# JuliaDiff/FiniteDiff.jl

Measured on AMD Instinct MI355X. Metric: Jacobian columns/s (coloured sparse finite-difference Jacobian; headline config N=10^7 tridiagonal forward), higher is better.
Workload: dtype f64; 1 GPU; N=10000000 tridiagonal CSC (nnz=3N-2), colorvec=mod1(i,3), forward, f!=second difference, x~U(0,1) seed 4; fdtype=forward, colors=3, parallelism=columns x1, output=nzval in HBM, eps_reduction=replicated, x_layout=replicated, gather_in_step=False

## Files before the change

finitediff.jl_amd/csrc/fdjac_builtin_f.hip:

```cpp
#include <atomic>
#include <cstdlib>
#include <mutex>
#include <new>
#include <unordered_map>
#include <vector>

#include "fdjac_internal.h"
#include "fdjac_eps_dev.h"

namespace fdjac {

constexpr real_t kTwo = 2, kFour = 4;
struct cd {
    real_t re, im;
};
__device__ __forceinline__ cd operator+(cd a, cd b) { return {a.re + b.re, a.im + b.im}; }
__device__ __forceinline__ cd operator-(cd a, cd b) { return {a.re - b.re, a.im - b.im}; }
__device__ __forceinline__ cd operator*(cd a, cd b) { return {a.re * b.re - a.im * b.im, a.re * b.im + a.im * b.re}; }
__device__ __forceinline__ cd operator*(real_t s, cd a) { return {s * a.re, s * a.im}; }
__device__ __forceinline__ cd operator+(cd a, real_t s) { return {a.re + s, a.im}; }
__device__ __forceinline__ cd operator-(cd a, real_t s) { return {a.re - s, a.im}; }

template <typename T> __device__ __forceinline__ T zero_of();
template <> __device__ __forceinline__ real_t zero_of<real_t>() { return 0.0; }
// ... 81 lines not shown
            xv[k] = in ? x[in ? j : 0] : 0.0;
            const int c = in ? (int)color[in ? j : 0] : -1;
            cv[k] = (c == (int)(CT)(-1) || c < 0) ? -1 : c - c_lo;
        }
        const bool two = i + 1 < n;
        real_t b0 = 0.0, b1 = 0.0;
        if (base_out || (diff && MODE == 0)) {
            b0 = tridiag_row<real_t, NL>(xv[0], xv[1], xv[2]);
            if (two) b1 = tridiag_row<real_t, NL>(xv[1], xv[2], xv[3]);
        }
        if (base_out) {
            if (two) *reinterpret_cast<r2_t *>(base_out + i) = r2_t{b0, b1};
            else base_out[i] = b0;
        }
        for (int b = 0; b < B; ++b) {
            const real_t e = eps[c_lo + b];
            real_t d[4];
#pragma unroll
            for (int k = 0; k < 4; ++k) d[k] = (cv[k] == b) ? e : 0.0;
            if (MODE == 2) {
                cd p[4];
#pragma unroll
                for (int k = 0; k < 4; ++k) p[k] = cd{xv[k], d[k]};
                const cd v0 = tridiag_row<cd, NL>(p[0], p[1], p[2]);
                if (imag_only) {
                    real_t *dst = fx + (int64_t)b * fs + i;
                    if (two) {
                        const cd v1 = tridiag_row<cd, NL>(p[1], p[2], p[3]);
                        *reinterpret_cast<r2_t *>(dst) = r2_t{v0.im, v1.im};
                    } else {
                        dst[0] = v0.im;
                    }
                } else {
                    real_t *dst = fx + ((int64_t)b * fs + i) * 2;
                    *reinterpret_cast<r2_t *>(dst) = r2_t{v0.re, v0.im};
                    if (two) {
                        const cd v1 = tridiag_row<cd, NL>(p[1], p[2], p[3]);
                        *reinterpret_cast<r2_t *>(dst + 2) = r2_t{v1.re, v1.im};
                    }
                }
            } else if (diff) {
                real_t p[4], q[4];
#pragma unroll
                for (int k = 0; k < 4; ++k) { p[k] = xv[k] + d[k]; q[k] = xv[k] - d[k]; }
                const real_t s0 = MODE == 1 ? tridiag_row<real_t, NL>(q[0], q[1], q[2]) : b0;
                const real_t v0 = sub_exact(tridiag_row<real_t, NL>(p[0], p[1], p[2]), s0);
                real_t v1 = 0.0;
                if (two) {
                    const real_t s1 = MODE == 1 ? tridiag_row<real_t, NL>(q[1], q[2], q[3]) : b1;
                    v1 = sub_exact(tridiag_row<real_t, NL>(p[1], p[2], p[3]), s1);
                }
                real_t *dst = fx + (int64_t)b * fs + i;
                if (two) *reinterpret_cast<r2_t *>(dst) = r2_t{v0, v1};
                else dst[0] = v0;
            } else {
#pragma unroll
                for (int sgn = 0; sgn < (MODE == 1 ? 2 : 1); ++sgn) {
                    real_t p[4];
#pragma unroll
                    for (int k = 0; k < 4; ++k) p[k] = sgn == 0 ? xv[k] + d[k] : xv[k] - d[k];
                    const real_t v0 = tridiag_row<real_t, NL>(p[0], p[1], p[2]);
                    real_t *dst = fx + (int64_t)(sgn * B + b) * fs + i;
                    if (two) {
                        const real_t v1 = tridiag_row<real_t, NL>(p[1], p[2], p[3]);
                        *reinterpret_cast<r2_t *>(dst) = r2_t{v0, v1};
                    } else {
                        dst[0] = v0;
                    }
                }
            }
        }
    }
}

__device__ __forceinline__ r2_t ld_pair_guarded(const real_t *__restrict__ x, int64_t a, int64_t n)
{
    if (a >= 0 && a + 1 < n) return *reinterpret_cast<const r2_t *>(x + a);
    r2_t v = {0, 0};
    if (a >= 0 && a < n) v.x = x[a];
    return v;
}

template <int MODE, bool NL>
__device__ __forceinline__ void tridiag_pair_quotients(const r2_t &L, const r2_t &Cc, const r2_t &R, real_t ea, real_t eb, real_t (&q)[6])
{
    const real_t xv[6] = {L.x, L.y, Cc.x, Cc.y, R.x, R.y};
#pragma unroll
    for (int o = 0; o < 2; ++o) {
        const real_t e = o == 0 ? ea : eb;
        const real_t ed = MODE == 1 ? 2 * e : e;
        real_t p[5], m[5];
#pragma unroll
        for (int k = 0; k < 5; ++k) { const real_t dlt = k == 2 ? e : (real_t)0; p[k] = xv[o + k] + dlt; m[k] = xv[o + k] - dlt; }
#pragma unroll
        for (int k = 0; k < 3; ++k) {
            const real_t plus = tridiag_row<real_t, NL>(p[k], p[k + 1], p[k + 2]);
            const real_t sub = MODE == 1 ? tridiag_row<real_t, NL>(m[k], m[k + 1], m[k + 2])
                                         : tridiag_row<real_t, NL>(xv[o + k], xv[o + k + 1], xv[o + k + 2]);
            q[3 * o + k] = sub_exact(plus, sub) / ed;
        }
    }
}

template <int MODE, bool NL>
__global__ void __launch_bounds__(kBlock)
k_f_tridiag_store_wave(const real_t *__restrict__ x, const real_t *__restrict__ eps, int64_t n, fd_band_store bst, int64_t jstart)
{
    __shared__ __attribute__((aligned(16))) real_t s_win[kBlock / 64][FD_BAND_WAVE_LDS(3)];
    const int lane = threadIdx.x & 63, wave = threadIdx.x >> 6;
    const int64_t nwaves = (bst.col_end - jstart + 127) / 128;
    const int64_t gw = (int64_t)blockIdx.x * (kBlock / 64) + wave;
    if (gw >= nwaves) return;
    const int64_t jw = jstart + gw * 128;
    const int64_t j = jw + 2 * lane;
    const r2_t Cc = ld_pair_guarded(x, j, n), L = ld_pair_guarded(x, j - 2, n), R = ld_pair_guarded(x, j + 2, n);
    const int c0w = (int)((jw + bst.shift) % bst.C);
    const int c0 = (int)((uint32_t)(c0w + 2 * lane) % (uint32_t)bst.C);
    const int c1 = c0 + 1 == bst.C ? 0 : c0 + 1;
    const real_t ea = eps[c0], eb = eps[c1];
    real_t q[6];
    tridiag_pair_quotients<MODE, NL>(L, Cc, R, ea, eb, q);
    fd_band_emit_wave<real_t, 3, true>(&bst, s_win[wave], jw, q);
}

template <int MODE, bool NL, int NC, bool PIPE>
__global__ void __launch_bounds__(kBlock)
k_f_tridiag_fused(const real_t *__restrict__ x, int64_t n, fd_band_store bst, int64_t jstart, FusedEps fz)
{
    constexpr int kWinBytes = (kBlock / 64) * FD_BAND_WAVE_LDS(3) * (int)sizeof(real_t);
    constexpr int kLdsBytes = kWinBytes + 64 > (kFzMaxBlocks + 2 * kEpsGroups) * 8 ? kWinBytes + 64 : (kFzMaxBlocks + 2 * kEpsGroups) * 8;
    __shared__ __attribute__((aligned(16))) char s_lds[kLdsBytes];
    real_t (*s_win)[FD_BAND_WAVE_LDS(3)] = reinterpret_cast<real_t (*)[FD_BAND_WAVE_LDS(3)]>(s_lds);
    double *s_red = reinterpret_cast<double *>(s_lds);
    const int b = (int)blockIdx.x, nfin = fz.eg.C;
    if (b < nfin) { fused_finisher(fz, b, s_red, x, n); return; }
    if (b < nfin + fz.nblocks) { fused_eps_block<NC, PIPE>(x, n, fz, b - nfin, reinterpret_cast<double (*)[NC]>(s_red)); return; }
    const int lane = threadIdx.x & 63, wave = threadIdx.x >> 6;
    const int cb = b - nfin - fz.nblocks;
    const int64_t nwaves = (bst.col_end - jstart + 127) / 128;
    const int64_t gstride = (int64_t)((int)gridDim.x - nfin - fz.nblocks) * (kBlock / 64);
    int64_t gw = (int64_t)cb * (kBlock / 64) + wave;
    int64_t jw = jstart + gw * 128;
    r2_t Cc = {0, 0}, L = {0, 0}, R = {0, 0};
    auto load_x = [&](int64_t jt, r2_t &c_, r2_t &l_, r2_t &r_) {
        const int64_t j = jt + 2 * lane;
        c_ = ld_pair_guarded(x, j, n); l_ = ld_pair_guarded(x, j - 2, n); r_ = ld_pair_guarded(x, j + 2, n);
        if (fz.xw && fz.nranks > 1) {
            if (j == fz.own_begin && fz.rank > 0) { l_.x = fused_halo(fz, 0, 0); l_.y = fused_halo(fz, 0, 1); }
            if (j + 2 == fz.own_end && fz.rank + 1 < fz.nranks) { r_.x = fused_halo(fz, 1, 0); r_.y = fused_halo(fz, 1, 1); }
        }
    };
    if (gw < nwaves) load_x(jw, Cc, L, R);
    real_t *s_eps = reinterpret_cast<real_t *>(s_lds + kWinBytes);
    if (wave == 0) fused_wait_eps(fz, cb, s_eps);
    __syncthreads();
    for (; gw < nwaves; gw += gstride) {
        const int c0w = (int)((jw + bst.shift) % bst.C);
        const int c0 = (int)((uint32_t)(c0w + 2 * lane) % (uint32_t)bst.C);
        const int c1 = c0 + 1 == bst.C ? 0 : c0 + 1;
        real_t q[6];
        tridiag_pair_quotients<MODE, NL>(L, Cc, R, s_eps[c0], s_eps[c1], q);
        fd_band_emit_wave<real_t, 3, true>(&bst, s_win[wave], jw, q);
        jw = jstart + (gw + gstride) * 128;
        if (gw + gstride < nwaves) load_x(jw, Cc, L, R);
    }
    if (fz.trace && (blockIdx.x & 31) < 2) { asm volatile("s_waitcnt vmcnt(0)" ::: "memory"); fz_mark_max(fz, 8); }
}

#ifdef FDJAC_F32
typedef real_t r4_t __attribute__((ext_vector_type(4)));
__device__ __forceinline__ r4_t ld_quad_guarded(const real_t *__restrict__ x, int64_t a, int64_t n)
{
    if (a >= 0 && a + 3 < n) return *reinterpret_cast<const r4_t *>(x + a);
    r4_t v = {0, 0, 0, 0};
    if (a >= 0 && a < n) v.x = x[a];
    if (a + 1 >= 0 && a + 1 < n) v.y = x[a + 1];
    if (a + 2 >= 0 && a + 2 < n) v.z = x[a + 2];
    if (a + 3 >= 0 && a + 3 < n) v.w = x[a + 3];
    return v;
}
template <int MODE, bool NL>
__device__ __forceinline__ void tridiag_quad_quotients(const r4_t &L, const r4_t &Cc, const r4_t &R, const real_t (&ev)[4], real_t (&q)[12])
{
    const real_t xv[8] = {L.z, L.w, Cc.x, Cc.y, Cc.z, Cc.w, R.x, R.y};
#pragma unroll
    for (int o = 0; o < 4; ++o) {
        const real_t e = ev[o];
        const real_t ed = MODE == 1 ? 2 * e : e;
        real_t p[5], m[5];
#pragma unroll
        for (int k = 0; k < 5; ++k) { const real_t dlt = k == 2 ? e : (real_t)0; p[k] = xv[o + k] + dlt; m[k] = xv[o + k] - dlt; }
#pragma unroll
        for (int k = 0; k < 3; ++k) {
            const real_t plus = tridiag_row<real_t, NL>(p[k], p[k + 1], p[k + 2]);
            const real_t sub = MODE == 1 ? tridiag_row<real_t, NL>(m[k], m[k + 1], m[k + 2])
                                         : tridiag_row<real_t, NL>(xv[o + k], xv[o + k + 1], xv[o + k + 2]);
            q[3 * o + k] = sub_exact(plus, sub) / ed;
        }
    }
}
template <int MODE, bool NL>
__global__ void __launch_bounds__(kBlock)
k_f_tridiag_store_wave4(const real_t *__restrict__ x, const real_t *__restrict__ eps, int64_t n, fd_band_store bst, int64_t jstart)
{
    __shared__ __attribute__((aligned(16))) real_t s_win[kBlock / 64][FD_BAND_WAVE4_LDS(3)];
    const int lane = threadIdx.x & 63, wave = threadIdx.x >> 6;
    const int64_t nwaves = (bst.col_end - jstart + 255) / 256;
    const int64_t gw = (int64_t)blockIdx.x * (kBlock / 64) + wave;
    if (gw >= nwaves) return;
    const int64_t jw = jstart + gw * 256;
    const int64_t j = jw + 4 * lane;
    const r4_t Cc = ld_quad_guarded(x, j, n), L = ld_quad_guarded(x, j - 4, n), R = ld_quad_guarded(x, j + 4, n);
    const int c0w = (int)((jw + bst.shift) % bst.C);
    int cc = (int)((uint32_t)(c0w + 4 * lane) % (uint32_t)bst.C);
    real_t ev[4];
#pragma unroll
    for (int o = 0; o < 4; ++o) { ev[o] = eps[cc]; cc = cc + 1 == bst.C ? 0 : cc + 1; }
    real_t q[12];
    tridiag_quad_quotients<MODE, NL>(L, Cc, R, ev, q);
    fd_band_emit_wave4<real_t, 3, true>(&bst, s_win[wave], jw, q);
}
template <int MODE, bool NL, int NC, bool PIPE>
__global__ void __launch_bounds__(kBlock)
k_f_tridiag_fused4(const real_t *__restrict__ x, int64_t n, fd_band_store bst, int64_t jstart, FusedEps fz)
{
    constexpr int kWinBytes = (kBlock / 64) * FD_BAND_WAVE4_LDS(3) * (int)sizeof(real_t);
    constexpr int kLdsBytes = kWinBytes + 64 > (kFzMaxBlocks + 2 * kEpsGroups) * 8 ? kWinBytes + 64 : (kFzMaxBlocks + 2 * kEpsGroups) * 8;
    __shared__ __attribute__((aligned(16))) char s_lds[kLdsBytes];
    real_t (*s_win)[FD_BAND_WAVE4_LDS(3)] = reinterpret_cast<real_t (*)[FD_BAND_WAVE4_LDS(3)]>(s_lds);
    double *s_red = reinterpret_cast<double *>(s_lds);
    const int b = (int)blockIdx.x, nfin = fz.eg.C;
    if (b < nfin) { fused_finisher(fz, b, s_red, x, n); return; }
    if (b < nfin + fz.nblocks) { fused_eps_block<NC, PIPE>(x, n, fz, b - nfin, reinterpret_cast<double (*)[NC]>(s_red)); return; }
    const int lane = threadIdx.x & 63, wave = threadIdx.x >> 6;
    const int cb = b - nfin - fz.nblocks;
    const int64_t nwaves = (bst.col_end - jstart + 255) / 256;
    const int64_t gstride = (int64_t)((int)gridDim.x - nfin - fz.nblocks) * (kBlock / 64);
    int64_t gw = (int64_t)cb * (kBlock / 64) + wave;
    int64_t jw = jstart + gw * 256;
    r4_t Cc = {0, 0, 0, 0}, L = {0, 0, 0, 0}, R = {0, 0, 0, 0};
    auto load_x = [&](int64_t jt, r4_t &c_, r4_t &l_, r4_t &r_) {
        const int64_t j = jt + 4 * lane;
        c_ = ld_quad_guarded(x, j, n); l_ = ld_quad_guarded(x, j - 4, n); r_ = ld_quad_guarded(x, j + 4, n);
        if (fz.xw && fz.nranks > 1) {
            if (j == fz.own_begin && fz.rank > 0) { l_.z = fused_halo(fz, 0, 0); l_.w = fused_halo(fz, 0, 1); }
// ... 390 lines not shown
    case FD_F_LAP5:
    case FD_F_LAP5_NL:
    case FD_F_CLAMP5: {
        const int sk = b->family == FD_F_CLAMP5 ? 1 : b->family == FD_F_LAP5_NL ? 2 : 0;
        if constexpr (sizeof(T) == sizeof(real_t)) {
            const bool ok = ((((uintptr_t)fx) | ((uintptr_t)x)) & kPairMask) == 0 && (xs % 2 == 0 || nbatch == 1) &&
                            (fs % 2 == 0 || nbatch == 1) && (b->prm[0] % 2 == 0);
            if (ok) {
                const int64_t r0e = r0 & ~(int64_t)1;
                const int64_t ntiles = (r1 - r0e + 2 * kBlock - 1) / (2 * kBlock);
                const dim3 g2((unsigned)(8 * xcd_chunks(ntiles)), (unsigned)nbatch, 1);
#define FD_ST_V2(SKK) hipLaunchKernelGGL((k_f_stencil5_v2<SKK>), g2, dim3(kBlock), 0, s, (real_t *)fx, (const real_t *)x, \
                                       b->prm[0], b->prm[1], xs, fs, r0e, r1)
                if (sk == 1) FD_ST_V2(1); else if (sk == 2) FD_ST_V2(2); else FD_ST_V2(0);
#undef FD_ST_V2
                break;
            }
        }
#define FD_ST(SKK) hipLaunchKernelGGL((k_f_stencil5<T, SKK>), g, dim3(kBlock), 0, s, fxp, xp, b->prm[0], b->prm[1], xs, fs, r0, r1)
        if (sk == 1) FD_ST(1); else if (sk == 2) FD_ST(2); else FD_ST(0);
#undef FD_ST
        break;
    }
    case FD_F_BLOCKCOUPLED: {
        const int64_t nb = b->prm[0], bs = b->prm[1];
        if (b->sig_cap < nbatch * nb) {
            if (b->d_sig) (void)hipFree(b->d_sig);
            b->d_sig = nullptr;
            if (hipMalloc(&b->d_sig, (size_t)(nbatch * nb) * 2 * sizeof(real_t)) != hipSuccess) return 2;
            b->sig_cap = nbatch * nb;
        }
        const int64_t b0 = std::max<int64_t>(r0 / bs - 1, 0), b1 = std::min<int64_t>((r1 + bs - 1) / bs + 1, nb);
        const dim3 gs = grid2((b1 - b0) * 64, nbatch, ncu);
        hipLaunchKernelGGL((k_f_block_sigma<T>), gs, dim3(kBlock), 0, s, (T *)b->d_sig, xp, nb, bs, xs, b0, b1);
        hipLaunchKernelGGL((k_f_block_apply<T>), g, dim3(kBlock), 0, s, fxp, xp, (const T *)b->d_sig, nb, bs, xs, fs, r0, r1);
        break;
    }
    case FD_F_NONSQUARE:
        hipLaunchKernelGGL((k_f_nonsquare<T>), g, dim3(kBlock), 0, s, fxp, xp, b->prm[0], xs, fs, r0, r1);
        break;
    default: return 3;
    }
    return hipGetLastError() == hipSuccess ? 0 : 4;
}

static int builtin_launch(void *fctx, void *fx, const void *x, int64_t nbatch, int64_t x_stride, int64_t fx_stride,
                          int64_t row_begin, int64_t row_end, int is_complex, void *stream)
{
    BuiltinF *b = (BuiltinF *)fctx;
    if (!b || b->magic != 0xFD0F00D5u) return 1;
    if (nbatch <= 0) return 0;
    if (nbatch > 65535) return 5;
    b->launches.fetch_add(1);
    b->points.fetch_add(nbatch);
    const int64_t r0 = std::max<int64_t>(row_begin, 0), r1 = std::min<int64_t>(row_end, b->M);
    if (is_complex)
        return launch_family<cd>(b, fx, x, nbatch, x_stride, fx_stride, r0, r1, (hipStream_t)stream);
    return launch_family<real_t>(b, fx, x, nbatch, x_stride, fx_stride, r0, r1, (hipStream_t)stream);
}

template <typename K>
static unsigned fused_grid(K kernel, unsigned tiles_wg, int prefix)
{
    static const int cus = [] { int dev = 0, n = 256; if (hipGetDevice(&dev) == hipSuccess) (void)hipDeviceGetAttribute(&n, hipDeviceAttributeMultiprocessorCount, dev); return n > 0 ? n : 256; }();
    static std::mutex mu;
    static std::unordered_map<const void *, int> per_cu;
    int occ = 0;
    {
        std::lock_guard<std::mutex> lock(mu);
        auto it = per_cu.find((const void *)kernel);
        if (it == per_cu.end()) {
            int nb = 0;
            if (hipOccupancyMaxActiveBlocksPerMultiprocessor(&nb, kernel, kBlock, 0) != hipSuccess || nb < 1) nb = 4;
            (void)hipGetLastError();
            it = per_cu.emplace((const void *)kernel, nb).first;
        }
        occ = it->second;
    }
    const int64_t room = (int64_t)cus * occ - prefix;
    const int64_t cap = room > cus ? room : cus;
    if ((int64_t)tiles_wg <= cap) return (unsigned)prefix + tiles_wg;
    const int64_t rounds = ((int64_t)tiles_wg + cap - 1) / cap;
    return (unsigned)prefix + (unsigned)(((int64_t)tiles_wg + rounds - 1) / rounds);
}

template <typename CT>
static int lazy_tridiag_launch(BuiltinF *b, void *fx, const fd_lazy_points *lp, int64_t fs, int64_t r0, int64_t r1,
                               hipStream_t s)
{
    const int64_t r0e = r0 & ~(int64_t)1;
    int64_t g = ((r1 - r0e + 1) / 2 + kBlock - 1) / kBlock;
    if (g < 1) g = 1;
    const bool nl = b->family == FD_F_TRIDIAG_NL;
    const int mode = lp->is_complex ? 2 : (lp->pts == 2 ? 1 : 0);
#define FD_LAZY(MODE, NL)                                                                                           \
    hipLaunchKernelGGL((k_f_tridiag_lazy<CT, MODE, NL>), dim3((unsigned)g), dim3(kBlock), 0, s, (real_t *)fx, fs,    \
                       (real_t *)lp->base_out, (const real_t *)lp->x, (const CT *)lp->color, (const real_t *)lp->eps, lp->c_lo,     \
                       lp->ncolors, b->prm[0], r0e, r1, lp->imag_only, mode != 2 ? lp->diff : 0)
    if (lp->store) {
        if (lp->store_kind != FD_STORE_BAND) return FD_LAZY_DECLINED;
        const fd_band_store bst = *(const fd_band_store *)lp->store;
        if (bst.elem_bytes != (int)sizeof(real_t) || mode == 2) return FD_LAZY_DECLINED;
        if (bst.N != b->prm[0] || bst.M != b->prm[0]) return FD_LAZY_DECLINED;
        const int wband = bst.l + bst.u + 1;
        const bool wave_ok = bst.l == 1 && bst.u == 1 && bst.M == bst.N && lp->c_lo == 0 &&
                             lp->ncolors == bst.C && bst.C >= 3 && (((uintptr_t)lp->x) & kPairMask) == 0 && bst.col_end > bst.col_begin;
#ifdef FDJAC_F32
        if (wave_ok && (((uintptr_t)lp->x) & 15) == 0) {
            const int64_t jstart = bst.col_begin & ~(int64_t)3;
            const int64_t nwaves = (bst.col_end - jstart + 255) / 256;
            const unsigned gw = (unsigned)((nwaves + kBlock / 64 - 1) / (kBlock / 64));
            if (lp->eps_job) {
                const FusedEps fz = *(const FusedEps *)lp->eps_job;
#define FD_LAZY_FZ4P(MODE, NL, NCC, PP) hipLaunchKernelGGL((k_f_tridiag_fused4<MODE, NL, NCC, PP>), dim3(fused_grid(k_f_tridiag_fused4<MODE, NL, NCC, PP>, gw, fz.eg.C + fz.nblocks)), dim3(kBlock), 0, s, (const real_t *)lp->x, b->prm[0], bst, jstart, fz)
#define FD_LAZY_FZ4(MODE, NL)                                                                                                              \
                do { if (fz.eg.C <= 4) { if (fz.eg.tpb > 2) FD_LAZY_FZ4P(MODE, NL, 4, true); else FD_LAZY_FZ4P(MODE, NL, 4, false); }               \
                     else { if (fz.eg.tpb > 2) FD_LAZY_FZ4P(MODE, NL, kRegColors, true); else FD_LAZY_FZ4P(MODE, NL, kRegColors, false); } } while (0)
                if (mode == 0) { if (nl) FD_LAZY_FZ4(0, true); else FD_LAZY_FZ4(0, false); }
                else { if (nl) FD_LAZY_FZ4(1, true); else FD_LAZY_FZ4(1, false); }
#undef FD_LAZY_FZ4
#undef FD_LAZY_FZ4P
                return hipGetLastError() == hipSuccess ? 0 : 4;
            }
#define FD_LAZY_SW4(MODE, NL)                                                                                      \
            hipLaunchKernelGGL((k_f_tridiag_store_wave4<MODE, NL>), dim3(gw), dim3(kBlock), 0, s, (const real_t *)lp->x, \
                               (const real_t *)lp->eps, b->prm[0], bst, jstart)
            if (mode == 0) { if (nl) FD_LAZY_SW4(0, true); else FD_LAZY_SW4(0, false); }
            else { if (nl) FD_LAZY_SW4(1, true); else FD_LAZY_SW4(1, false); }
#undef FD_LAZY_SW4
            return hipGetLastError() == hipSuccess ? 0 : 4;
        }
#endif
        if (wave_ok) {
            const int64_t jstart = bst.col_begin & ~(int64_t)1;
            const int64_t nwaves = (bst.col_end - jstart + 127) / 128;
            const unsigned gw = (unsigned)((nwaves + kBlock / 64 - 1) / (kBlock / 64));
            if (lp->eps_job) {
                const FusedEps fz = *(const FusedEps *)lp->eps_job;
#define FD_LAZY_FZP(MODE, NL, NCC, PP) hipLaunchKernelGGL((k_f_tridiag_fused<MODE, NL, NCC, PP>), dim3(fused_grid(k_f_tridiag_fused<MODE, NL, NCC, PP>, gw, fz.eg.C + fz.nblocks)), dim3(kBlock), 0, s, (const real_t *)lp->x, b->prm[0], bst, jstart, fz)
#define FD_LAZY_FZ(MODE, NL)                                                                                                              \
                do { if (fz.eg.C <= 4) { if (fz.eg.tpb > 2) FD_LAZY_FZP(MODE, NL, 4, true); else FD_LAZY_FZP(MODE, NL, 4, false); }               \
                     else { if (fz.eg.tpb > 2) FD_LAZY_FZP(MODE, NL, kRegColors, true); else FD_LAZY_FZP(MODE, NL, kRegColors, false); } } while (0)
                if (mode == 0) { if (nl) FD_LAZY_FZ(0, true); else FD_LAZY_FZ(0, false); }
                else { if (nl) FD_LAZY_FZ(1, true); else FD_LAZY_FZ(1, false); }
#undef FD_LAZY_FZ
#undef FD_LAZY_FZP
                return hipGetLastError() == hipSuccess ? 0 : 4;
            }
#define FD_LAZY_SW(MODE, NL)                                                                                       \
            hipLaunchKernelGGL((k_f_tridiag_store_wave<MODE, NL>), dim3(gw), dim3(kBlock), 0, s, (const real_t *)lp->x,  \
                               (const real_t *)lp->eps, b->prm[0], bst, jstart)
            if (mode == 0) { if (nl) FD_LAZY_SW(0, true); else FD_LAZY_SW(0, false); }
            else { if (nl) FD_LAZY_SW(1, true); else FD_LAZY_SW(1, false); }
#undef FD_LAZY_SW
            return hipGetLastError() == hipSuccess ? 0 : 4;
        }
        if (lp->eps_job) return FD_LAZY_DECLINED;
        if (bst.layout != FD_BAND_CSC) return FD_LAZY_DECLINED;
        const int bs = kBlock;
        const int pitch = 2 * bs + 2;
        const size_t shm = sizeof(real_t) * ((size_t)lp->ncolors * (size_t)pitch + (size_t)lp->ncolors + 2);
        const int64_t nnz_all = fd_band_colptr(&bst, bst.N);
        if (shm > (size_t)60 * 1024 || nnz_all + (int64_t)wband * wband + 64 >= ((int64_t)1 << 31) || bst.N + bst.C + 64 >= ((int64_t)1 << 31) ||
            bst.M + wband + 64 >= ((int64_t)1 << 31) || lp->ncolors > kBlock) return FD_LAZY_DECLINED;
        const unsigned gs = (unsigned)((r1 - r0e + 2 * bs - 1) / (2 * bs));
#define FD_LAZY_ST(MODE, NL)                                                                                       \
        hipLaunchKernelGGL((k_f_tridiag_lazy_store<CT, MODE, NL, kBlock>), dim3(gs), dim3(kBlock), shm, s, (const real_t *)lp->x, \
                           (const CT *)lp->color, (const real_t *)lp->eps, lp->c_lo, lp->ncolors, (int)b->prm[0], (int)r0e, (int)r1, \
                           (real_t *)bst.out, (int)bst.M, (int)bst.N, (int)bst.entry_begin, (int)bst.col_begin, (int)bst.col_end,     \
                           bst.l, bst.u, bst.C, bst.shift, pitch, fd_magic31((uint32_t)wband), fd_magic31((uint32_t)bst.C))
        if (mode == 0) { if (nl) FD_LAZY_ST(0, true); else FD_LAZY_ST(0, false); }
        else { if (nl) FD_LAZY_ST(1, true); else FD_LAZY_ST(1, false); }
#undef FD_LAZY_ST
        return hipGetLastError() == hipSuccess ? 0 : 4;
    }
    if (mode == 0) { if (nl) FD_LAZY(0, true); else FD_LAZY(0, false); }
    else if (mode == 1) { if (nl) FD_LAZY(1, true); else FD_LAZY(1, false); }
    else { if (nl) FD_LAZY(2, true); else FD_LAZY(2, false); }
#undef FD_LAZY
    return hipGetLastError() == hipSuccess ? 0 : 4;
}

template <typename T, int SK> __device__ __forceinline__ T stencil5_row(T c, T w, T e, T s, T n)
{
    T v = (((w + e) + s) + n) - kFour * c;
    if (SK == 2) v = v + (c * c) * e;
    return v;
}

__device__ __forceinline__ bool div_shared_ok(real_t b) { const real_t mb = fabs(b); return mb >= (real_t)0x1p-100 && mb <= (real_t)0x1p100; }
__device__ __forceinline__ bool div_is_pow2(real_t b)
{
    if constexpr (sizeof(real_t) == 8) {
        const unsigned long long u = (unsigned long long)__double_as_longlong((double)b), ex = (u >> 52) & 0x7FFull;
        return (u & 0x000FFFFFFFFFFFFFull) == 0 && ex >= 2 && ex <= 2044;
    } else {
        const unsigned u = __float_as_uint((float)b), ex = (u >> 23) & 0xFFu;
        return (u & 0x007FFFFFu) == 0 && ex >= 2 && ex <= 252;
    }
}
template <bool FAST> __device__ __forceinline__ real_t div_shared(real_t a, real_t b, real_t y);
template <bool FAST> __device__ __forceinline__ real_t div_shared(real_t a, real_t b, real_t y, bool bok)
{
    if constexpr (FAST && sizeof(real_t) == 8) {
        const double ma = fabs(a);
        if (!(bok && ma >= 0x1p-800 && ma <= 0x1p800)) return a / b;
        const double q0 = a * y;
        const double r0 = __builtin_fma(-b, q0, a);
        const double q1 = __builtin_fma(r0, y, q0);
        const double r1 = __builtin_fma(-b, q1, a);
        return __builtin_fma(r1, y, q1);
    } else {
        return a / b;
    }
}
template <bool FAST> __device__ __forceinline__ real_t div_shared(real_t a, real_t b, real_t y)
{
    if constexpr (FAST && sizeof(real_t) == 8) {
        const double q0 = a * y;
        const double m = fabs(q0), ma = fabs(a);
        if (!(m >= 0x1p-900 && m <= 0x1p900 && ma >= 0x1p-900 && ma <= 0x1p900)) return a / b;
        const double r0 = __builtin_fma(-b, q0, a);
        const double q1 = __builtin_fma(r0, y, q0);
        const double r1 = __builtin_fma(-b, q1, a);
        return __builtin_fma(r1, y, q1);
    } else {
        return a / b;
    }
}

template <int MODE, int SK, bool INTERIOR, bool FASTDIV, int WC, bool NUMER = false, bool YGIVEN = false>
__device__ __forceinline__ void stencil5_column_quotients(const real_t (&W)[5][WC], int o, int ii, int j, int nx, int ny, real_t e, real_t *q,
                                                          real_t yd_in = 0)
{
// ... 1282 lines not shown
```

include/fdjac_device.h:

```cpp
#ifndef FDJAC_DEVICE_H
#define FDJAC_DEVICE_H

#if defined(__HIPCC__)
#define FD_DEVICE_FN __host__ __device__ static inline
#else
#define FD_DEVICE_FN static inline
#endif

enum fd_band_layout {
    FD_BAND_CSC = 0,
    FD_BAND_BANDED = 1,
    FD_BAND_TRIDIAGONAL = 2
};

typedef struct fd_band_store {
    void *out;
    long long M, N;
    long long entry_begin;
    long long col_begin, col_end;
    int l, u;
    int C, shift;
    int layout;
    int elem_bytes;
    void *out_dl, *out_du;
// ... 139 lines not shown
        if (r == 0) for (long long k = 1; k <= d->u - j; ++k) ((T *)d->out)[at - k] = (T)0;
        if (r == d->M - 1) for (long long k = 1; k <= j + d->l - (d->M - 1); ++k) ((T *)d->out)[at + k] = (T)0;
    }
}

template <typename T> __device__ inline void fd_band_emit_column(const fd_band_store *d, long long j, const T *q)
{
    if (j < d->col_begin || j >= d->col_end || j < 0 || j >= d->N) return;
    const int w = d->l + d->u + 1;
    if (d->layout == FD_BAND_TRIDIAGONAL) {
        const long long du0 = d->col_begin > 0 ? d->col_begin - 1 : 0;
        if (j > 0) ((T *)d->out_du)[j - 1 - du0] = q[0];
        ((T *)d->out)[j - d->col_begin] = q[1];
        if (j + 1 < d->M) ((T *)d->out_dl)[j - d->col_begin] = q[2];
        return;
    }
    if (d->layout == FD_BAND_BANDED) {
        T *o = (T *)d->out + (long long)w * (j - d->col_begin);
        for (int k = 0; k < w; ++k) { const long long r = j - d->u + k; o[k] = (r >= 0 && r < d->M) ? q[k] : (T)0; }
        return;
    }
    const long long first = j - d->u > 0 ? j - d->u : 0;
    T *o = (T *)d->out + (fd_band_colptr(d, j) - d->entry_begin) - (first - (j - d->u));
    for (int k = 0; k < w; ++k) { const long long r = j - d->u + k; if (r >= 0 && r < d->M) o[k] = q[k]; }
}

#define FD_BAND_WAVE_LDS(W) (128 * (W) + 8)

template <typename T> struct fd_band_pair_of;
template <> struct fd_band_pair_of<double> { typedef double type __attribute__((ext_vector_type(2))); };
template <> struct fd_band_pair_of<float> { typedef float type __attribute__((ext_vector_type(2))); };

template <typename T, int W, bool NT = true>
__device__ inline void fd_band_emit_wave(const fd_band_store *d, T *win, long long jw, const T *q)
{
    typedef typename fd_band_pair_of<T>::type pair_t;
    const int lane = (int)(threadIdx.x & 63);
    const long long j = jw + 2 * lane;
    const long long jlast = jw + 127;
    const bool inside = jw >= d->col_begin && jlast < d->col_end && jlast < d->N;
    bool fast = inside && d->layout != FD_BAND_TRIDIAGONAL && ((((unsigned long long)d->out) & (2 * sizeof(T) - 1)) == 0);
    if (d->layout == FD_BAND_CSC) fast = fast && jw >= d->u && jlast + d->l <= d->M - 1;
    if (d->layout == FD_BAND_BANDED) fast = fast && jw >= d->u && jlast + d->l <= d->M - 1;
    if (W == 3 && d->layout == FD_BAND_TRIDIAGONAL && inside && jw >= 1 && jlast + 1 <= d->M - 1) {
        T *pd = (T *)d->out + (j - d->col_begin), *pl = (T *)d->out_dl + (j - d->col_begin);
        const long long du0 = d->col_begin > 0 ? d->col_begin - 1 : 0;
        T *pu = (T *)d->out_du + (j - du0);
        const T nq0 = __shfl_down(q[0], 1, 64);
        const T q1 = q[1], q2 = q[2], q3 = q[W], q4 = q[W + 1], q5 = q[W + 2];
        if ((((unsigned long long)pd) & (2 * sizeof(T) - 1)) == 0) __builtin_nontemporal_store(pair_t{q1, q4}, (pair_t *)pd);
        else { pd[0] = q1; pd[1] = q4; }
        if ((((unsigned long long)pl) & (2 * sizeof(T) - 1)) == 0) __builtin_nontemporal_store(pair_t{q2, q5}, (pair_t *)pl);
        else { pl[0] = q2; pl[1] = q5; }
        if (lane == 0) pu[-1] = q[0];
        if (lane < 63 && (((unsigned long long)pu) & (2 * sizeof(T) - 1)) == 0) __builtin_nontemporal_store(pair_t{q3, nq0}, (pair_t *)pu);
        else { pu[0] = q3; if (lane < 63) pu[1] = nq0; }
        return;
    }
    if (!fast) {
        fd_band_emit_column<T>(d, j, q);
        fd_band_emit_column<T>(d, j + 1, q + W);
        return;
    }
    const long long P0 = d->layout == FD_BAND_BANDED ? (long long)W * (jw - d->col_begin)
                                                     : (long long)W * jw - (long long)d->u * (d->u + 1) / 2 - d->entry_begin;
    const int off = (int)(P0 & 1);
#pragma unroll
    for (int m = 0; m < 2 * W; ++m) win[off + 2 * W * lane + m] = q[m];
    __builtin_amdgcn_fence(__ATOMIC_RELEASE, "wavefront");
    __builtin_amdgcn_wave_barrier();
    __builtin_amdgcn_fence(__ATOMIC_ACQUIRE, "wavefront");
    T *base = (T *)d->out + (P0 - off);
#pragma unroll
    for (int a = 0; a < W; ++a) {
        const int sl = 2 * (64 * a + lane);
        const pair_t v = *(const pair_t *)(win + sl);
        if (off && sl == 0) base[1] = v.y;
        else if (NT) __builtin_nontemporal_store(v, (pair_t *)(base + sl));
        else *(pair_t *)(base + sl) = v;
    }
    if (off && lane == 63) base[128 * W] = q[2 * W - 1];
    __builtin_amdgcn_fence(__ATOMIC_RELEASE, "wavefront");
    __builtin_amdgcn_wave_barrier();
}
#define FD_BAND_WAVE4_LDS(W) (256 * (W) + 8)
template <typename T> struct fd_band_quad_of;
template <> struct fd_band_quad_of<float> { typedef float type __attribute__((ext_vector_type(4))); };
template <> struct fd_band_quad_of<double> { typedef double type __attribute__((ext_vector_type(4))); };
template <typename T, int W, bool NT = true>
__device__ inline void fd_band_emit_wave4(const fd_band_store *d, T *win, long long jw, const T *q)
{
    typedef typename fd_band_quad_of<T>::type quad_t;
    const int lane = (int)(threadIdx.x & 63);
    const long long j = jw + 4 * lane;
    const long long jlast = jw + 255;
    const bool inside = jw >= d->col_begin && jlast < d->col_end && jlast < d->N;
    const unsigned long long qmask = 4 * sizeof(T) - 1;
    bool fast = inside && d->layout != FD_BAND_TRIDIAGONAL && ((((unsigned long long)d->out) & qmask) == 0) &&
                jw >= d->u && jlast + d->l <= d->M - 1;
    if (W == 3 && d->layout == FD_BAND_TRIDIAGONAL && inside && jw >= 1 && jlast + 1 <= d->M - 1) {
        T *pd = (T *)d->out + (j - d->col_begin), *pl = (T *)d->out_dl + (j - d->col_begin);
        const long long du0 = d->col_begin > 0 ? d->col_begin - 1 : 0;
        T *pu = (T *)d->out_du + (j - du0);
        const T nq0 = __shfl_down(q[0], 1, 64);
        const quad_t vd = {q[1], q[W + 1], q[2 * W + 1], q[3 * W + 1]}, vl = {q[2], q[W + 2], q[2 * W + 2], q[3 * W + 2]};
        const quad_t vu = {q[W], q[2 * W], q[3 * W], nq0};
        if ((((unsigned long long)pd) & qmask) == 0) { if (NT) __builtin_nontemporal_store(vd, (quad_t *)pd); else *(quad_t *)pd = vd; }
        else { pd[0] = vd.x; pd[1] = vd.y; pd[2] = vd.z; pd[3] = vd.w; }
        if ((((unsigned long long)pl) & qmask) == 0) { if (NT) __builtin_nontemporal_store(vl, (quad_t *)pl); else *(quad_t *)pl = vl; }
        else { pl[0] = vl.x; pl[1] = vl.y; pl[2] = vl.z; pl[3] = vl.w; }
        if (lane == 0) pu[-1] = q[0];
        if (lane < 63 && (((unsigned long long)pu) & qmask) == 0) { if (NT) __builtin_nontemporal_store(vu, (quad_t *)pu); else *(quad_t *)pu = vu; }
        else { pu[0] = vu.x; pu[1] = vu.y; pu[2] = vu.z; if (lane < 63) pu[3] = vu.w; }
        return;
    }
    if (!fast) {
#pragma unroll
        for (int c = 0; c < 4; ++c) fd_band_emit_column<T>(d, j + c, q + c * W);
        return;
    }
    const long long P0 = d->layout == FD_BAND_BANDED ? (long long)W * (jw - d->col_begin)
                                                     : (long long)W * jw - (long long)d->u * (d->u + 1) / 2 - d->entry_begin;
    const int off = (int)(P0 & 3);
#pragma unroll
    for (int m = 0; m < 4 * W; ++m) win[off + 4 * W * lane + m] = q[m];
    __builtin_amdgcn_fence(__ATOMIC_RELEASE, "wavefront");
    __builtin_amdgcn_wave_barrier();
    __builtin_amdgcn_fence(__ATOMIC_ACQUIRE, "wavefront");
    T *base = (T *)d->out + (P0 - off);
#pragma unroll
    for (int a = 0; a < W; ++a) {
        const int sl = 4 * (64 * a + lane);
        const quad_t v = *(const quad_t *)(win + sl);
        if (off && sl == 0) {
            if (off <= 1) base[1] = v.y;
            if (off <= 2) base[2] = v.z;
            base[3] = v.w;
        } else if (NT) __builtin_nontemporal_store(v, (quad_t *)(base + sl));
        else *(quad_t *)(base + sl) = v;
    }
    if (lane < off) base[256 * W + lane] = win[256 * W + lane];
    __builtin_amdgcn_fence(__ATOMIC_RELEASE, "wavefront");
    __builtin_amdgcn_wave_barrier();
}

template <typename T, bool NT> __device__ inline void fd_wave_store_window(T *base, const T *win, int lo, int hi)
{
    typedef typename fd_band_pair_of<T>::type pair_t;
    const int lane = (int)(threadIdx.x & 63);
    for (int sl = 2 * lane; sl < hi; sl += 128) {
        const bool l0 = sl >= lo, l1 = sl + 1 < hi;
        if (l0 && l1) {
            const pair_t v = *(const pair_t *)(win + sl);
            if (NT) __builtin_nontemporal_store(v, (pair_t *)(base + sl));
            else *(pair_t *)(base + sl) = v;
        } else {
            if (l0) base[sl] = win[sl];
            if (l1 && sl + 1 >= lo) base[sl + 1] = win[sl + 1];
        }
    }
}

template <typename T> __device__ inline void fd_stencil5_emit_column_ij(const fd_stencil5_store *d, long long i, long long j, const T *q)
{
    const long long k = j * d->nx + i;
    if (k < d->col_begin || k >= d->col_end) return;
// ... 1137 lines not shown
```

Baseline: 148.5 billion columns/s.

## Align tridiagonal wave stores to 128-byte lines with a shifted output window

Adds a CSC store path in which each wave writes a contiguous run of 384 nzval entries starting at a shifted entry offset, rather than the column-aligned window. To fill the gap it recomputes the first quotient of the next column in lane 63. The start column is chosen from the output pointer and entry_begin so that each wave's stores begin on a 16-element (128-byte) boundary, aiming for full cache-line writes. It is enabled by default and can be turned off with an env switch. Boundary waves fall back to per-column stores, which adds complexity and some duplicated arithmetic.

```diff
diff --git a/finitediff.jl_amd/csrc/fdjac_builtin_f.hip b/finitediff.jl_amd/csrc/fdjac_builtin_f.hip
--- a/finitediff.jl_amd/csrc/fdjac_builtin_f.hip
+++ b/finitediff.jl_amd/csrc/fdjac_builtin_f.hip
@@ -187,29 +187,42 @@
 }
 
 template <int MODE, bool NL>
+__device__ __forceinline__ real_t tridiag_quotient(const real_t *xv, real_t e, int k)
+{
+    const real_t ed = MODE == 1 ? 2 * e : e;
+    real_t p[3], m[3];
+#pragma unroll
+    for (int i = 0; i < 3; ++i) { const real_t dlt = k + i == 2 ? e : (real_t)0; p[i] = xv[k + i] + dlt; m[i] = xv[k + i] - dlt; }
+    const real_t plus = tridiag_row<real_t, NL>(p[0], p[1], p[2]);
+    const real_t sub = MODE == 1 ? tridiag_row<real_t, NL>(m[0], m[1], m[2]) : tridiag_row<real_t, NL>(xv[k], xv[k + 1], xv[k + 2]);
+    return sub_exact(plus, sub) / ed;
+}
+
+template <int MODE, bool NL>
 __device__ __forceinline__ void tridiag_pair_quotients(const r2_t &L, const r2_t &Cc, const r2_t &R, real_t ea, real_t eb, real_t (&q)[6])
 {
     const real_t xv[6] = {L.x, L.y, Cc.x, Cc.y, R.x, R.y};
 #pragma unroll
-    for (int o = 0; o < 2; ++o) {
-        const real_t e = o == 0 ? ea : eb;
-        const real_t ed = MODE == 1 ? 2 * e : e;
-        real_t p[5], m[5];
-#pragma unroll
-        for (int k = 0; k < 5; ++k) { const real_t dlt = k == 2 ? e : (real_t)0; p[k] = xv[o + k] + dlt; m[k] = xv[o + k] - dlt; }
-#pragma unroll
-        for (int k = 0; k < 3; ++k) {
-            const real_t plus = tridiag_row<real_t, NL>(p[k], p[k + 1], p[k + 2]);
-            const real_t sub = MODE == 1 ? tridiag_row<real_t, NL>(m[k], m[k + 1], m[k + 2])
-                                         : tridiag_row<real_t, NL>(xv[o + k], xv[o + k + 1], xv[o + k + 2]);
-            q[3 * o + k] = sub_exact(plus, sub) / ed;
-        }
-    }
+    for (int o = 0; o < 2; ++o)
+#pragma unroll
+        for (int k = 0; k < 3; ++k) q[3 * o + k] = tridiag_quotient<MODE, NL>(xv + o, o == 0 ? ea : eb, k);
+}
+template <int MODE, bool NL>
+__device__ __forceinline__ real_t tridiag_next_quotient(const r2_t &Cc, const r2_t &R, real_t en)
+{
+    const real_t xv[3] = {Cc.x, Cc.y, R.x};
+    return tridiag_quotient<MODE, NL>(xv, en, 0);
+}
+
+__device__ __forceinline__ int tridiag_wave_color(int64_t jw, const fd_band_store &bst)
+{
+    const int64_t m = (jw + bst.shift) % bst.C;
+    return (int)(m < 0 ? m + bst.C : m);
 }
 
 template <int MODE, bool NL>
 __global__ void __launch_bounds__(kBlock)
-k_f_tridiag_store_wave(const real_t *__restrict__ x, const real_t *__restrict__ eps, int64_t n, fd_band_store bst, int64_t jstart)
+k_f_tridiag_store_wave(const real_t *__restrict__ x, const real_t *__restrict__ eps, int64_t n, fd_band_store bst, int64_t jstart, int lines)
 {
     __shared__ __attribute__((aligned(16))) real_t s_win[kBlock / 64][FD_BAND_WAVE_LDS(3)];
     const int lane = threadIdx.x & 63, wave = threadIdx.x >> 6;
@@ -219,18 +232,25 @@
     const int64_t jw = jstart + gw * 128;
     const int64_t j = jw + 2 * lane;
     const r2_t Cc = ld_pair_guarded(x, j, n), L = ld_pair_guarded(x, j - 2, n), R = ld_pair_guarded(x, j + 2, n);
-    const int c0w = (int)((jw + bst.shift) % bst.C);
+    const int c0w = tridiag_wave_color(jw, bst);
     const int c0 = (int)((uint32_t)(c0w + 2 * lane) % (uint32_t)bst.C);
     const int c1 = c0 + 1 == bst.C ? 0 : c0 + 1;
     const real_t ea = eps[c0], eb = eps[c1];
+    const real_t en = lines ? eps[(uint32_t)(c0w + 128) % (uint32_t)bst.C] : (real_t)0;
     real_t q[6];
     tridiag_pair_quotients<MODE, NL>(L, Cc, R, ea, eb, q);
+    if (lines) {
+        real_t qn = 0;
+        if (lane == 63) qn = tridiag_next_quotient<MODE, NL>(Cc, R, en);
+        fd_band_emit_wave_lines<real_t, true>(&bst, s_win[wave], jw, q, qn);
+        return;
+    }
     fd_band_emit_wave<real_t, 3, true>(&bst, s_win[wave], jw, q);
 }
 
 template <int MODE, bool NL, int NC, bool PIPE>
 __global__ void __launch_bounds__(kBlock)
-k_f_tridiag_fused(const real_t *__restrict__ x, int64_t n, fd_band_store bst, int64_t jstart, FusedEps fz)
+k_f_tridiag_fused(const real_t *__restrict__ x, int64_t n, fd_band_store bst, int64_t jstart, int lines, FusedEps fz)
 {
     constexpr int kWinBytes = (kBlock / 64) * FD_BAND_WAVE_LDS(3) * (int)sizeof(real_t);
     constexpr int kLdsBytes = kWinBytes + 64 > (kFzMaxBlocks + 2 * kEpsGroups) * 8 ? kWinBytes + 64 : (kFzMaxBlocks + 2 * kEpsGroups) * 8;
@@ -260,12 +280,18 @@
     if (wave == 0) fused_wait_eps(fz, cb, s_eps);
     __syncthreads();
     for (; gw < nwaves; gw += gstride) {
-        const int c0w = (int)((jw + bst.shift) % bst.C);
+        const int c0w = tridiag_wave_color(jw, bst);
         const int c0 = (int)((uint32_t)(c0w + 2 * lane) % (uint32_t)bst.C);
         const int c1 = c0 + 1 == bst.C ? 0 : c0 + 1;
         real_t q[6];
         tridiag_pair_quotients<MODE, NL>(L, Cc, R, s_eps[c0], s_eps[c1], q);
-        fd_band_emit_wave<real_t, 3, true>(&bst, s_win[wave], jw, q);
+        if (lines) {
+            real_t qn = 0;
+            if (lane == 63) qn = tridiag_next_quotient<MODE, NL>(Cc, R, s_eps[(uint32_t)(c0w + 128) % (uint32_t)bst.C]);
+            fd_band_emit_wave_lines<real_t, true>(&bst, s_win[wave], jw, q, qn);
+        } else {
+            fd_band_emit_wave<real_t, 3, true>(&bst, s_win[wave], jw, q);
+        }
         jw = jstart + (gw + gstride) * 128;
         if (gw + gstride < nwaves) load_x(jw, Cc, L, R);
     }
@@ -822,6 +848,20 @@
     if ((int64_t)tiles_wg <= cap) return (unsigned)prefix + tiles_wg;
     const int64_t rounds = ((int64_t)tiles_wg + cap - 1) / cap;
     return (unsigned)prefix + (unsigned)(((int64_t)tiles_wg + rounds - 1) / rounds);
+}
+
+static bool tridiag_lines_jstart(const fd_band_store &bst, int64_t *jstart)
+{
+    if (sizeof(real_t) != 8 || bst.layout != FD_BAND_CSC) return false;
+    const char *sw = fdjac::test_switch("FDJAC_STORE_LINES");
+    if (sw && *sw && atoi(sw) == 0) return false;
+    const uintptr_t o = (uintptr_t)bst.out;
+    if (o & 7) return false;
+    const int64_t r = (int64_t)(((uint64_t)bst.entry_begin - (uint64_t)(o >> 3)) & 15);
+    const int64_t want = (11 * r) & 15;
+    if (want & 1) return false;
+    *jstart -= (*jstart - want) & 15;
+    return true;
 }
 
 template <typename CT>
@@ -872,12 +912,13 @@
         }
 #endif
         if (wave_ok) {
-            const int64_t jstart = bst.col_begin & ~(int64_t)1;
+            int64_t jstart = bst.col_begin & ~(int64_t)1;
+            const int lines = tridiag_lines_jstart(bst, &jstart) ? 1 : 0;
             const int64_t nwaves = (bst.col_end - jstart + 127) / 128;
             const unsigned gw = (unsigned)((nwaves + kBlock / 64 - 1) / (kBlock / 64));
             if (lp->eps_job) {
                 const FusedEps fz = *(const FusedEps *)lp->eps_job;
-#define FD_LAZY_FZP(MODE, NL, NCC, PP) hipLaunchKernelGGL((k_f_tridiag_fused<MODE, NL, NCC, PP>), dim3(fused_grid(k_f_tridiag_fused<MODE, NL, NCC, PP>, gw, fz.eg.C + fz.nblocks)), dim3(kBlock), 0, s, (const real_t *)lp->x, b->prm[0], bst, jstart, fz)
+#define FD_LAZY_FZP(MODE, NL, NCC, PP) hipLaunchKernelGGL((k_f_tridiag_fused<MODE, NL, NCC, PP>), dim3(fused_grid(k_f_tridiag_fused<MODE, NL, NCC, PP>, gw, fz.eg.C + fz.nblocks)), dim3(kBlock), 0, s, (const real_t *)lp->x, b->prm[0], bst, jstart, lines, fz)
 #define FD_LAZY_FZ(MODE, NL)                                                                                                              \
                 do { if (fz.eg.C <= 4) { if (fz.eg.tpb > 2) FD_LAZY_FZP(MODE, NL, 4, true); else FD_LAZY_FZP(MODE, NL, 4, false); }               \
                      else { if (fz.eg.tpb > 2) FD_LAZY_FZP(MODE, NL, kRegColors, true); else FD_LAZY_FZP(MODE, NL, kRegColors, false); } } while (0)
@@ -889,7 +930,7 @@
             }
 #define FD_LAZY_SW(MODE, NL)                                                                                       \
             hipLaunchKernelGGL((k_f_tridiag_store_wave<MODE, NL>), dim3(gw), dim3(kBlock), 0, s, (const real_t *)lp->x,  \
-                               (const real_t *)lp->eps, b->prm[0], bst, jstart)
+                               (const real_t *)lp->eps, b->prm[0], bst, jstart, lines)
             if (mode == 0) { if (nl) FD_LAZY_SW(0, true); else FD_LAZY_SW(0, false); }
             else { if (nl) FD_LAZY_SW(1, true); else FD_LAZY_SW(1, false); }
 #undef FD_LAZY_SW
diff --git a/include/fdjac_device.h b/include/fdjac_device.h
--- a/include/fdjac_device.h
+++ b/include/fdjac_device.h
@@ -245,6 +245,47 @@
     if (off && lane == 63) base[128 * W] = q[2 * W - 1];
     __builtin_amdgcn_fence(__ATOMIC_RELEASE, "wavefront");
     __builtin_amdgcn_wave_barrier();
+}
+__device__ inline bool fd_band_wave_lines(const fd_band_store *d, long long jw)
+{
+    return d->layout == FD_BAND_CSC && jw >= 1 && jw > d->col_begin && jw + 128 < d->col_end && jw + 128 < d->N && jw + 128 < d->M;
+}
+template <typename T, bool NT = true>
+__device__ inline void fd_band_emit_wave_lines(const fd_band_store *d, T *win, long long jw, const T *q, T qnext)
+{
+    typedef typename fd_band_pair_of<T>::type pair_t;
+    const int lane = (int)(threadIdx.x & 63);
+    const long long E = 3 * jw - d->entry_begin;
+    if (fd_band_wave_lines(d, jw)) {
+        if (lane) win[6 * lane - 1] = q[0];
+#pragma unroll
+        for (int m = 1; m < 6; ++m) win[6 * lane + m - 1] = q[m];
+        if (lane == 63) win[383] = qnext;
+        __builtin_amdgcn_fence(__ATOMIC_RELEASE, "wavefront");
+        __builtin_amdgcn_wave_barrier();
+        __builtin_amdgcn_fence(__ATOMIC_ACQUIRE, "wavefront");
+        T *base = (T *)d->out + E;
+#pragma unroll
+        for (int a = 0; a < 3; ++a) {
+            const int sl = 2 * (64 * a + lane);
+            const pair_t v = *(const pair_t *)(win + sl);
+            if (NT) __builtin_nontemporal_store(v, (pair_t *)(base + sl));
+            else *(pair_t *)(base + sl) = v;
+        }
+        __builtin_amdgcn_fence(__ATOMIC_RELEASE, "wavefront");
+        __builtin_amdgcn_wave_barrier();
+        return;
+    }
+    const long long j = jw + 2 * lane;
+    if (lane == 0 && fd_band_wave_lines(d, jw - 128)) {
+        T *o = (T *)d->out + E;
+        o[0] = q[1];
+        if (jw + 1 < d->M) o[1] = q[2];
+    } else {
+        fd_band_emit_column<T>(d, j, q);
+    }
+    fd_band_emit_column<T>(d, j + 1, q + 3);
+    if (lane == 63 && fd_band_wave_lines(d, jw + 128)) ((T *)d->out)[E + 383] = qnext;
 }
 #define FD_BAND_WAVE4_LDS(W) (256 * (W) + 8)
 template <typename T> struct fd_band_quad_of;
```

Result: faster. 151.3 billion columns/s (median of 6 runs) (+1.9%).
